# Nerozud/dl_reference_models

Hardware: NVIDIA B200
Metric: agent_steps_per_sec (higher is better)
Workload: dtype int16/u8

## Files before the change

dl_reference_models_b200/csrc/mapf_env_kernel.cuh:

```cuda
#pragma once

#include "mapf_kernels.cuh"

namespace mapf {

constexpr int ENV_MAX_ROWS = 64;
constexpr int ENV_T1_OFF = 0;
constexpr int ENV_KTH_OFF = 512;
constexpr int ENV_FREEROW_OFF = 768;
constexpr int ENV_FREEBITS_OFF = 1024;
constexpr int ENV_GDT_OFF = 1280;
constexpr int ENV_LUT_OFF = 2048;
constexpr int ENV_ROW_PAD = 2;

__host__ __device__ constexpr int env_stage_stride(int V2) { return ((4 * V2 + 20 + 3) / 4) | 1; }
__host__ __device__ constexpr int env_stage_bytes(int V2) {
    return 32 * env_stage_stride(V2) * 4 > 32 * 64 ? 32 * env_stage_stride(V2) * 4 : 32 * 64;
}

struct EnvLayout {
    int tables_bytes;
    int pre_off;
    int warp_bytes;
    int board_rows;
    int nq;
    int total_bytes;
};

__host__ __device__ inline EnvLayout make_env_layout(int N, int R, int C, int SR, int fw, int warps) {
    const int V = 2 * SR + 1, V2 = V * V;
    EnvLayout E;
    E.pre_off = (ENV_LUT_OFF + R * 32 * (V > 5 ? 8 : 4) + 15) & ~15;
    E.tables_bytes = E.pre_off + 65 * 4 + 12;
    E.board_rows = R > C ? R : C;
    if (N > E.board_rows) E.board_rows = N;
    E.board_rows += 2 * ENV_ROW_PAD;
    E.nq = (N + 3) / 4;
    int w = env_stage_bytes(V2);
    w += E.board_rows * 32 * 4;
    w += E.board_rows * 32 * 4;
    w += 4 * E.nq * 32 * 4;
    w = (w + 15) & ~15;
    E.warp_bytes = w;
    E.total_bytes = E.tables_bytes + w * warps + 1024;
    (void)fw;
    return E;
}

template <bool VEC>
__device__ __forceinline__ uint4 ldq32(const uint32_t *a, size_t i, int i0, int N, bool ok, uint32_t d) {
    uint4 v = make_uint4(d, d, d, d);
    if (VEC) { if (ok) v = *reinterpret_cast<const uint4 *>(a + i); }
    else if (ok) {
        if (i0 + 0 < N) v.x = a[i + 0];
        if (i0 + 1 < N) v.y = a[i + 1];
        if (i0 + 2 < N) v.z = a[i + 2];
        if (i0 + 3 < N) v.w = a[i + 3];
    }
    return v;
}
template <bool VEC>
__device__ __forceinline__ void stq32(uint32_t *a, size_t i, int i0, int N, bool ok, uint4 v) {
    if (!ok) return;
    if (VEC) *reinterpret_cast<uint4 *>(a + i) = v;
    else {
        if (i0 + 0 < N) a[i + 0] = v.x;
        if (i0 + 1 < N) a[i + 1] = v.y;
        if (i0 + 2 < N) a[i + 2] = v.z;
        if (i0 + 3 < N) a[i + 3] = v.w;
    }
}
template <bool VEC>
__device__ __forceinline__ uint32_t ldq8(const uint8_t *a, size_t i, int i0, int N, bool ok) {
    uint32_t v = 0;
    if (VEC) { if (ok) v = *reinterpret_cast<const uint32_t *>(a + i); }
    else if (ok) {
#pragma unroll
        for (int k = 0; k < 4; ++k) if (i0 + k < N) v |= (uint32_t)a[i + k] << (8 * k);
    }
    return v;
}
template <bool VEC>
__device__ __forceinline__ void stq8(uint8_t *a, size_t i, int i0, int N, bool ok, uint32_t v) {
    if (!ok) return;
    if (VEC) *reinterpret_cast<uint32_t *>(a + i) = v;
    else {
#pragma unroll
        for (int k = 0; k < 4; ++k) if (i0 + k < N) a[i + k] = (uint8_t)(v >> (8 * k));
    }
}
template <bool VEC>
__device__ __forceinline__ uint2 ldq16(const int16_t *a, size_t i, int i0, int N, bool ok) {
    uint2 v = make_uint2(0, 0);
    if (VEC) { if (ok) v = *reinterpret_cast<const uint2 *>(a + i); }
    else if (ok) {
        if (i0 + 0 < N) v.x |= (uint32_t)(uint16_t)a[i + 0];
        if (i0 + 1 < N) v.x |= (uint32_t)(uint16_t)a[i + 1] << 16;
        if (i0 + 2 < N) v.y |= (uint32_t)(uint16_t)a[i + 2];
        if (i0 + 3 < N) v.y |= (uint32_t)(uint16_t)a[i + 3] << 16;
    }
    return v;
}
template <bool VEC>
__device__ __forceinline__ void stq16(int16_t *a, size_t i, int i0, int N, bool ok, uint2 v) {
    if (!ok) return;
    if (VEC) *reinterpret_cast<uint2 *>(a + i) = v;
    else {
        if (i0 + 0 < N) a[i + 0] = (int16_t)(v.x & 0xFFFFu);
        if (i0 + 1 < N) a[i + 1] = (int16_t)(v.x >> 16);
        if (i0 + 2 < N) a[i + 2] = (int16_t)(v.y & 0xFFFFu);
        if (i0 + 3 < N) a[i + 3] = (int16_t)(v.y >> 16);
    }
}

__device__ __forceinline__ uint32_t qget(const uint4 &v, int k) { return k == 0 ? v.x : k == 1 ? v.y : k == 2 ? v.z : v.w; }
__device__ __forceinline__ void qset(uint4 &v, int k, uint32_t x) { if (k == 0) v.x = x; else if (k == 1) v.y = x; else if (k == 2) v.z = x; else v.w = x; }
__device__ __forceinline__ uint32_t hget(const uint2 &v, int k) { const uint32_t w = (k < 2) ? v.x : v.y; return (k & 1) ? (w >> 16) : (w & 0xFFFFu); }
__device__ __forceinline__ void hset(uint2 &v, int k, uint32_t x) {
    uint32_t &w = (k < 2) ? v.x : v.y;
    w = (k & 1) ? ((w & 0x0000FFFFu) | (x << 16)) : ((w & 0xFFFF0000u) | (x & 0xFFFFu));
}
__device__ __forceinline__ uint32_t code_of(uint32_t packed) { return ((packed & 0xFFFFu) << 5) | (packed >> 16); }
__device__ __forceinline__ uint32_t packed_of(uint32_t code) { return (code >> 5) | ((code & 31u) << 16); }

__device__ __forceinline__ uint4 sample_quad(unsigned long long seed, long long env_global, int quad,
                                             unsigned long long counter) {
    Philox ph(seed ^ 0xA511E9B3ull, env_global);
    return ph((uint32_t)counter, (uint32_t)(counter >> 32), (uint32_t)quad, 0x41435421u);
}

inline void build_env_tables(int SR, int R, int C, int wpr, int fw, const uint32_t *rows,
                             const uint32_t *free_bits, int normalize, float den0, float den1, unsigned char *img,
                             int pre_off) {
    const int V = 2 * SR + 1;
    {
        uint32_t *pre = reinterpret_cast<uint32_t *>(img + pre_off);
        uint32_t acc = 0;
        for (int w = 0; w <= 64; ++w) {
            pre[w] = acc;
            if (w < fw) acc += (uint32_t)__builtin_popcount(free_bits[w]);
        }
    }
    auto rowbits = [&](int r, int c0, int n) {
        unsigned long long x = 0;
        for (int j = 0; j < n; ++j) {
            const int bit = c0 + j + PAD;
            if ((rows[(r + PAD) * wpr + (bit >> 5)] >> (bit & 31)) & 1u) x |= 1ull << j;
        }
        return x;
    };
    uint32_t *t1 = reinterpret_cast<uint32_t *>(img + ENV_T1_OFF);
    for (int x = 0; x < (1 << V); ++x) {
        uint32_t s = 0;
        for (int j = 0; j < V; ++j) s |= ((uint32_t)(x >> j) & 1u) << (4 * j);
        t1[x] = s;
    }
    uint8_t *kth = img + ENV_KTH_OFF;
    for (int m = 0; m < 32; ++m)
        for (int k = 0; k < 8; ++k) {
            int pos = 0, seen = 0;
            for (int b = 0; b < 5; ++b)
                if ((m >> b) & 1) { if (seen == k) pos = b; ++seen; }
            kth[m * 8 + k] = (uint8_t)(k < seen ? pos : 0);
        }
    for (int cell = 0; cell < R * 32; ++cell) {
        const int r = cell >> 5, c = cell & 31;
        unsigned long long w = 0;
        if (c < C)
            for (int wr = 0; wr < V; ++wr) w |= rowbits(r - SR + wr, c - SR, V) << (wr * V);
        if (V > 5) reinterpret_cast<unsigned long long *>(img + ENV_LUT_OFF)[cell] = w;
        else reinterpret_cast<uint32_t *>(img + ENV_LUT_OFF)[cell] = (uint32_t)w;
    }
    uint32_t *freerow = reinterpret_cast<uint32_t *>(img + ENV_FREEROW_OFF);
    for (int r = 0; r < R; ++r) freerow[r] = (uint32_t)(~rowbits(r, 0, C) & (C >= 32 ? 0xFFFFFFFFull : ((1ull << C) - 1ull)));
    uint32_t *fb = reinterpret_cast<uint32_t *>(img + ENV_FREEBITS_OFF);
    for (int i = 0; i < fw; ++i) fb[i] = free_bits[i];
    float *gdt = reinterpret_cast<float *>(img + ENV_GDT_OFF);
    const int nr = 2 * R - 1, n = nr + 2 * C - 1;
    for (int i = 0; i < n; ++i) {
        const bool row = i < nr;
        const float d = (float)(row ? i - (R - 1) : i - nr - (C - 1));
        gdt[i] = normalize ? d / (row ? den0 : den1) : d;
    }
}

__device__ __forceinline__ uint32_t nibbles_to_bytes(uint32_t sel) {
    uint32_t w;
    asm("prmt.b32 %0, %1, %2, %3;" : "=r"(w) : "r"(0x03020100u), "r"(0x00000004u), "r"(sel));
    return w;
}
__device__ __forceinline__ uint32_t nibbles_to_bytes_0124(uint32_t sel) {
    uint32_t w;
    asm("prmt.b32 %0, %1, %2, %3;" : "=r"(w) : "r"(0x04020100u), "r"(0u), "r"(sel));
    return w;
}
__device__ __forceinline__ uint32_t spread4(uint32_t m) { return ((m & 15u) * 0x00204081u) & 0x01010101u; }
__device__ __forceinline__ uint32_t gather4(uint32_t w, int b) { return ((((w >> b) & 0x01010101u) * 0x01020408u) >> 24) & 15u; }
__device__ __forceinline__ int action_delta(uint32_t a) { return (int)(int8_t)__byte_perm(0x2001E000u, 0x000000FFu, a); }
__device__ __forceinline__ uint32_t lds_pure(uint32_t saddr) {
    uint32_t v;
    asm("ld.shared.u32 %0, [%1];" : "=r"(v) : "r"(saddr));
    return v;
}
__device__ __forceinline__ uint32_t lds_pure(uint32_t saddr, uint32_t tag) {
    uint32_t v;
    asm("{ .reg .b32 t; mov.b32 t, %2; ld.shared.u32 %0, [%1]; }" : "=r"(v) : "r"(saddr), "r"(tag));
    return v;
}
__device__ __forceinline__ uint32_t lds_pure_u8(uint32_t saddr) {
    uint32_t v;
    asm("ld.shared.u8 %0, [%1];" : "=r"(v) : "r"(saddr));
    return v;
}
template <typename WB> __device__ __forceinline__ WB lut_ld(uint32_t saddr);
template <> __device__ __forceinline__ uint32_t lut_ld<uint32_t>(uint32_t saddr) { return lds_pure(saddr); }
template <> __device__ __forceinline__ unsigned long long lut_ld<unsigned long long>(uint32_t saddr) {
    unsigned long long v;
    asm("ld.shared.u64 %0, [%1];" : "=l"(v) : "r"(saddr));
    return v;
}
__device__ __forceinline__ void sts_stage(uint32_t saddr, uint32_t v) {
    asm volatile("st.shared.u32 [%0], %1;" ::"r"(saddr), "r"(v));
}

__device__ __forceinline__ void sts_stage_u8(uint32_t saddr, uint32_t v) {
    asm volatile("st.shared.u8 [%0], %1;" ::"r"(saddr), "r"(v));
}

constexpr uint32_t REC_CODE = 0x7FFu;

template <int SR, bool VEC, bool FAST = false, bool MANY = false>
__global__ void __launch_bounds__(448, 1) mapf_step_env_kernel(const KParams p, const EnvLayout E) {
    const bool kLifelong = FAST ? true : p.lifelong;
    const bool kLock = FAST ? true : p.lock_enabled;
    constexpr int V = 2 * SR + 1, V2 = V * V;
    constexpr uint32_t VM = (1u << V) - 1u;
    constexpr uint32_t M4 = VM << 2;
    constexpr int OBS_W = V2;
    constexpr int STRIDE = env_stage_stride(V2);
    constexpr int STAGE_BYTES = env_stage_bytes(V2);
    constexpr int CTR = SR * V + SR;
    constexpr int PADR = ENV_ROW_PAD;
    using WB = typename WinBits<V>::type;
    extern __shared__ __align__(16) unsigned char esm[];
    const unsigned full = 0xFFFFFFFFu;
    const int tid = threadIdx.x, lane = tid & 31, warp = tid >> 5, warps = blockDim.x >> 5;
    const int N = p.N, R = p.R, C = p.C, NQ = E.nq;

    {
        const uint4 *src = reinterpret_cast<const uint4 *>(p.env_tables);
        uint4 *dst = reinterpret_cast<uint4 *>(esm);
        for (int i = tid; i < (E.tables_bytes >> 4); i += blockDim.x) dst[i] = src[i];
    }
    asm volatile("griddepcontrol.launch_dependents;");
    if (p.env_prefetch) {
        const int tile0 = blockIdx.x * (blockDim.x >> 5) + (tid >> 5);
        const int left = p.B - tile0 * 32;
        if (left > 0) {
            const size_t a0 = (size_t)tile0 * 32 * (size_t)p.N;
            const uint32_t agents = (uint32_t)(left < 32 ? left : 32) * (uint32_t)p.N;
            const void *ptr = nullptr;
            uint32_t bytes = agents * 4u;
            switch (tid & 31) {
                case 0: ptr = p.positions + a0; break;
                case 1: ptr = p.goals + a0; break;
                case 2: ptr = p.lock_gp + a0; break;
                case 3: ptr = p.lock_mv + a0; break;
                case 4: ptr = p.lock_fm + a0; break;
                case 5: ptr = p.actions ? p.actions + a0 : nullptr; bytes = agents; break;
                case 6: ptr = p.agent_flags + a0; bytes = agents; break;
                case 7: ptr = p.env_words + (size_t)tile0 * 32 * 4; bytes = (uint32_t)(left < 32 ? left : 32) * 64u; break;
                default: break;
            }
            bytes &= ~15u;
            if (ptr && bytes && (reinterpret_cast<uintptr_t>(ptr) & 15) == 0)
                asm volatile("cp.async.bulk.prefetch.L2.global [%0], %1;" ::"l"(ptr), "r"(bytes) : "memory");
        }
    }
    asm volatile("griddepcontrol.wait;" ::: "memory");
    __syncthreads();
    const char *t1b = reinterpret_cast<const char *>(esm + ENV_T1_OFF);
    const uint8_t *kth = esm + ENV_KTH_OFF;
    const WB *lut = reinterpret_cast<const WB *>(esm + ENV_LUT_OFF);
    const uint32_t *freerow = reinterpret_cast<const uint32_t *>(esm + ENV_FREEROW_OFF);
    const uint32_t *freebits = reinterpret_cast<const uint32_t *>(esm + ENV_FREEBITS_OFF);
    const float *gdt = reinterpret_cast<const float *>(esm + ENV_GDT_OFF);
    const uint32_t esm_s = (uint32_t)__cvta_generic_to_shared(esm);
    const uint32_t t1_s = esm_s + ENV_T1_OFF, kth_s = esm_s + ENV_KTH_OFF, lut_s = esm_s + ENV_LUT_OFF;
    const uint32_t *freepre = reinterpret_cast<const uint32_t *>(esm + E.pre_off);
    auto kth_free = [&](int k) -> int {
        int lo = 0;
#pragma unroll
        for (int stp = 32; stp >= 1; stp >>= 1)
            if (lo + stp < p.fw && (int)freepre[lo + stp] <= k) lo += stp;
        return lo * 32 + (int)__fns(freebits[lo], 0, k - (int)freepre[lo] + 1);
    };

    unsigned char *wsm = esm + E.tables_bytes + warp * E.warp_bytes;
    uint32_t *stage_w = reinterpret_cast<uint32_t *>(wsm);
    uint32_t *my_stage = stage_w + lane * STRIDE;
    const uint32_t my_stage_s = (uint32_t)__cvta_generic_to_shared(my_stage);
    uint32_t *occ_w = reinterpret_cast<uint32_t *>(wsm + STAGE_BYTES);
    uint32_t *goal_w = occ_w + E.board_rows * 32;
    uint32_t *rec_w = goal_w + E.board_rows * 32;
    uint32_t *occ = occ_w + lane, *goalb = goal_w + lane, *rec = rec_w + lane;
    const uint32_t goalb_s = (uint32_t)__cvta_generic_to_shared(goalb);
    uint32_t *rowm = occ, *colm = goalb;
    const int ntiles = (p.B + 31) / 32;
    uint32_t errs = 0;
    const uint32_t mdw = p.dw >= 32 ? full : ((1u << p.dw) - 1u);
    const uint32_t mlw = p.lw >= 32 ? full : ((1u << p.lw) - 1u);
    const uint32_t allN = (N >= 32) ? full : ((1u << N) - 1u);

    auto emit_final = [&](size_t abe, size_t oo, unsigned long long sctr, long long eg, const uint32_t *occ_e,
                          const uint32_t *goal_e, uint32_t code, uint32_t gcode, uint32_t bp_bit, bool ctr2) {
        if (lane >= N) return;
        const int r = (int)(code >> 5), c = (int)(code & 31u);
        const WB obst = lut[code];
        const int sa = c > SR ? c - SR : 0, sb2 = (c < SR ? SR - c : 0) + 2;
        const uint32_t *orow = occ_e + (r - SR) * 32, *grow = goal_e + (r - SR) * 32;
        uint32_t acc[(4 * V2 + 31) / 32 + 1];
#pragma unroll
        for (int j = 0; j < (int)(sizeof(acc) / sizeof(acc[0])); ++j) acc[j] = 0;
        uint32_t blk_up = 0, blk_mid = 0, blk_dn = 0;
#pragma unroll
        for (int wr = 0; wr < V; ++wr) {
            const uint32_t bx = orow[wr * 32], by = grow[wr * 32];
            const uint32_t o4 = (wr * V >= 2 ? (uint32_t)(obst >> (wr * V - 2)) : (uint32_t)(obst << 2)) & M4;
            const uint32_t MC = (wr == SR) ? (M4 & ~(4u << SR)) : M4;
            const uint32_t occ4 = ((bx >> sa) << sb2) & MC;
            const uint32_t agent4 = occ4 & ~o4, blk4 = occ4 | o4;
            const uint32_t g4 = ((by >> sa) << sb2) & M4 & ~blk4;
            if (wr == SR - 1) blk_up = blk4;
            if (wr == SR) blk_mid = blk4;
            if (wr == SR + 1) blk_dn = blk4;
            const uint32_t t = *reinterpret_cast<const uint32_t *>(t1b + o4) +
                               (*reinterpret_cast<const uint32_t *>(t1b + agent4) << 1) +
                               (*reinterpret_cast<const uint32_t *>(t1b + g4) << 2);
            const int bitpos = 4 * V * wr, wi = bitpos >> 5, sh = bitpos & 31;
            acc[wi] |= t << sh;
            if (sh + 4 * V > 32) acc[wi + 1] |= t >> (32 - sh);
        }
        const uint32_t am = 1u | ((~blk_up >> (2 + SR)) & 1u) << 1 | ((~blk_mid >> (2 + SR + 1)) & 1u) << 2 |
                            ((~blk_dn >> (2 + SR)) & 1u) << 3 | ((~blk_mid >> (2 + SR - 1)) & 1u) << 4;
        if (p.o_local_obs) {
            uint8_t *ob = p.o_local_obs + (abe + oo + lane) * V2;
#pragma unroll
            for (int n = 0; n < V2; ++n) ob[n] = (uint8_t)((acc[n >> 3] >> (4 * (n & 7))) & 0xFu);
            const int dr = (int)(gcode >> 5) - r + SR, dc = (int)(gcode & 31u) - c + SR;
            if ((unsigned)dr < (unsigned)V && (unsigned)dc < (unsigned)V) {
                const int ci = dr * V + dc;
                const bool occ_other = (ci != CTR) && ((occ_e[(gcode >> 5) * 32] >> (gcode & 31u)) & 1u);
                if (!((obst >> ci) & 1) && !occ_other) ob[ci] = 3;
            }
            if (ctr2) ob[CTR] = 2;
        }
        if (p.o_action_mask) {
#pragma unroll
            for (int k = 0; k < 5; ++k) p.o_action_mask[(abe + oo + lane) * 5 + k] = (int8_t)((am >> k) & 1u);
        }
        if (p.o_goal_delta) {
            const int gi0 = (int)(gcode >> 5) - r + (R - 1), gi1 = (int)(gcode & 31u) - c + (C - 1) + 2 * R - 1;
            p.o_goal_delta[abe + oo + lane] = make_float2(gdt[gi0], gdt[gi1]);
        }
        if (p.o_blocking_prev) p.o_blocking_prev[abe + oo + lane] = (uint8_t)bp_bit;
        if (p.sample_mode) {
            const uint4 rnd = sample_quad(p.seed, eg, lane >> 2, sctr);
            const uint32_t x = qget(rnd, lane & 3);
            const uint32_t na = p.sample_mode == 1 ? kth[am * 8 + __umulhi(x, (uint32_t)__popc(am))] : __umulhi(x, 5u);
            p.o_next_actions[abe + lane] = (int8_t)na;
        }
    };

    for (int tile = blockIdx.x * warps + warp; tile < ntiles; tile += gridDim.x * warps) {
    const int env = tile * 32 + lane;
    const bool ok = env < p.B;
    const size_t ab = (size_t)(ok ? env : 0) * N;
    const long long env_global = p.env_id_base + env;
    const size_t env0 = (size_t)tile * 32;
    for (int it = 0; it < (MANY ? p.inner_steps : 1); ++it) {
    const size_t so = MANY ? (size_t)it * (size_t)p.out_step_stride : 0, oo = so * (size_t)N;
    const unsigned long long sctr = p.sample_counter + (MANY ? (unsigned long long)it : 0ull);
    const int8_t *acts_in = (MANY && it > 0) ? p.o_next_actions : p.actions;

    int lock_count = 0, lock_head = 0;
    if (ok) {
        const int *ew1 = reinterpret_cast<const int *>(p.env_words + (size_t)env * 4);
        lock_count = ew1[MAPF_W_LOCK_COUNT];
        lock_head = ew1[MAPF_W_LOCK_HEAD];
    }
    const int count_after = lock_count + 1;
    if (lock_head < 0 || lock_head >= p.lw) lock_head = 0;
    const int slot_new = lock_head;
    const int slot_next = (lock_head + 1 == p.lw) ? 0 : lock_head + 1;
    const bool use_ring = kLock && count_after >= p.lw && p.lw > 1;

    uint32_t reached_m = 0, completed_m = 0, bprev_m = 0;
    bool degen = false;
    uint32_t solo_m = 0xFFFFFFFFu;
    for (int r = 0; r < E.board_rows; ++r) { occ[r * 32] = 0u; goalb[r * 32] = 0u; }
    uint32_t dup = 0;
    auto prepass_quad = [&](int i0, const uint4 &pq, const uint4 &gq, uint32_t act4, uint32_t fl4) {
        reached_m |= gather4(fl4, 0) << i0;
        completed_m |= gather4(fl4, 1) << i0;
        bprev_m |= gather4(fl4, 2) << i0;
        solo_m &= ~(gather4(fl4, 3) << i0);
#pragma unroll
        for (int k = 0; k < 4; ++k) {
            if (VEC || i0 + k < N) {
                const uint32_t code = code_of(qget(pq, k)), gcode = code_of(qget(gq, k));
                int a = (int)(int8_t)(act4 >> (8 * k));
                if (a < 0 || a > 4) { errs |= MAPF_DEV_ERR_INVALID_ACTION; a = 0; }
                const uint32_t nbi = __byte_perm((uint32_t)CTR | ((uint32_t)(CTR - V) << 8) | ((uint32_t)(CTR + 1) << 16) |
                                                 ((uint32_t)(CTR + V) << 24), (uint32_t)(CTR - 1), (uint32_t)a) & 0xFFu;
                const uint32_t tblocked = ((uint32_t)lut[code] >> nbi) & 1u;
                rec[(i0 + k) * 32] = code | ((uint32_t)a << 11) | (tblocked << 14) | (gcode << 16);
                if (ok) {
                    if (!((fl4 >> (8 * k + 3)) & 1u)) {
                        const uint32_t cb0 = 1u << (code & 31u);
                        dup |= atomicOr(&occ[(code >> 5) * 32], cb0) & cb0;
                    } else degen = true;
                    atomicOr(&goalb[(gcode >> 5) * 32], 1u << (gcode & 31u));
                }
            }
        }
    };
    for (int q = 0; q < NQ; q += 2) {
        const int i0 = 4 * q, i1 = i0 + 4;
        const bool two = q + 1 < NQ;
        const uint4 pq0 = ldq32<VEC>(p.positions, ab + i0, i0, N, ok, 0u);
        const uint4 gq0 = ldq32<VEC>(p.goals, ab + i0, i0, N, ok, 0u);
        const uint32_t ac0 = acts_in ? ldq8<VEC>(reinterpret_cast<const uint8_t *>(acts_in), ab + i0, i0, N, ok) : 0u;
        const uint32_t fl0 = ldq8<VEC>(p.agent_flags, ab + i0, i0, N, ok);
        const uint4 pq1 = ldq32<VEC>(p.positions, ab + i1, i1, N, ok && two, 0u);
        const uint4 gq1 = ldq32<VEC>(p.goals, ab + i1, i1, N, ok && two, 0u);
        const uint32_t ac1 = acts_in ? ldq8<VEC>(reinterpret_cast<const uint8_t *>(acts_in), ab + i1, i1, N, ok && two) : 0u;
        const uint32_t fl1 = ldq8<VEC>(p.agent_flags, ab + i1, i1, N, ok && two);
        prepass_quad(i0, pq0, gq0, ac0, fl0);
        if (two) prepass_quad(i1, pq1, gq1, ac1, fl1);
    }
    degen |= dup != 0;
    if (degen) {
        const uint32_t claim = solo_m;
        for (int i = 0; i < N; ++i)
            for (int j = i + 1; j < N; ++j)
                if (((claim >> j) & 1u) && ((rec[i * 32] ^ rec[j * 32]) & REC_CODE) == 0u) { solo_m &= ~(1u << i); break; }
    }

    uint32_t moved_m = 0, failed_m = 0, gstep_m = 0, ongoal_m = 0;
    uint32_t Gd = 0, Md = 0, Fd = 0, Gl = 0, Ml = 0;
    const unsigned act_w = __ballot_sync(full, ok);
    const bool masked_sampler = p.sample_mode == 1;

    uint4 gp_n = make_uint4(0, 0, 0, 0), mv_n = gp_n, fm_n = gp_n;
    uint2 ring_n = make_uint2(0u, 0u);
    auto load_lock = [&](int i0) {
        if (!kLock) return;
        gp_n = ldq32<VEC>(p.lock_gp, ab + i0, i0, N, ok, 0u);
        mv_n = ldq32<VEC>(p.lock_mv, ab + i0, i0, N, ok, 0u);
        fm_n = ldq32<VEC>(p.lock_fm, ab + i0, i0, N, ok, 0u);
        if (use_ring) ring_n = ldq16<VEC>(p.lock_dist, ((size_t)(ok ? env : 0) * p.lw + slot_next) * N + i0, i0, N, ok);
    };
    load_lock(0);
    for (int q = 0; q < NQ; ++q) {
        const int i0 = 4 * q;
        uint32_t rv4[4];
#pragma unroll
        for (int k = 0; k < 4; ++k) rv4[k] = (VEC || i0 + k < N) ? rec[(i0 + k) * 32] : 0u;
        uint4 gpq = gp_n, mvq = mv_n, fmq = fm_n;
        const uint2 ringq = ring_n;
        uint4 rnd = make_uint4(0, 0, 0, 0);
        if (p.sample_mode) rnd = sample_quad(p.seed, env_global, q, sctr);
        uint32_t ds[4] = {0, 0, 0, 0}, cd[4] = {0, 0, 0, 0}, gc[4] = {0, 0, 0, 0};
        uint32_t masks4 = 0, next4 = 0;
        int patch[4];
        uint32_t win[4][V];
#pragma unroll
        for (int k = 0; k < 4; ++k) {
            patch[k] = 4 * V2 + 20;
#pragma unroll
            for (int wr = 0; wr < V; ++wr) win[k][wr] = 0;
            if (!VEC && i0 + k >= N) continue;
            const uint32_t bit = 1u << (i0 + k);
            uint32_t code = rv4[k] & REC_CODE;
            const uint32_t gcode = rv4[k] >> 16;
            const uint32_t ocode = code;
            const uint32_t a = (rv4[k] >> 11) & 7u;
            const uint32_t tcode = code + (uint32_t)action_delta(a);
            const bool wants = ok && a != 0 && !(rv4[k] & 0x4000u);
            const uint32_t tb = 1u << (tcode & 31u);
            const uint32_t tv = occ[(tcode >> 5) * 32];
            const bool moves = wants & ((tv & tb) == 0u);
            atomicAnd(&occ[(code >> 5) * 32], moves ? ~(1u << (code & 31u)) : 0xFFFFFFFFu);
            atomicOr(&occ[(tcode >> 5) * 32], moves ? tb : 0u);
            const bool failed = ok && a != 0 && !moves;
            moved_m |= moves ? bit : 0u;
            failed_m |= failed ? bit : 0u;
            code = moves ? tcode : code;
            const bool on_goal = ok && code == gcode;
            bool gstep = false, cur_on_goal = on_goal;
            if (!kLifelong) {
                if (on_goal && !(reached_m & bit)) { reached_m |= bit; completed_m |= bit; gstep = true; }
            } else if (on_goal) {
                gstep = true;
                completed_m |= bit; reached_m &= ~bit;
                cur_on_goal = false;
            }
            gstep_m |= gstep ? bit : 0u;
            ongoal_m |= cur_on_goal ? bit : 0u;
            uint32_t delta16 = 0;
            if (kLock) {
                const bool prev_on_goal = kLifelong ? false : (ocode == gcode);
                const bool gp = kLifelong ? gstep : (!prev_on_goal && cur_on_goal);
                const uint32_t g2 = (qget(gpq, k) << 1) | (gp ? 1u : 0u);
                const uint32_t m2 = (qget(mvq, k) << 1) | (moves ? 1u : 0u);
                const uint32_t f2 = (qget(fmq, k) << 1) | (failed ? 1u : 0u);
                qset(gpq, k, g2); qset(mvq, k, m2); qset(fmq, k, f2);
                const uint32_t okbit = ok ? bit : 0u;
                Gd |= (g2 & mdw) ? okbit : 0u;
                Md |= (m2 & mdw) ? okbit : 0u;
                Fd |= (f2 & mdw) ? okbit : 0u;
                Gl |= (g2 & mlw) ? okbit : 0u;
                Ml |= (m2 & mlw) ? okbit : 0u;
                const int dist = abs((int)(gcode >> 5) - (int)(code >> 5)) + abs((int)(gcode & 31u) - (int)(code & 31u));
                ds[k] = (uint32_t)dist;
                delta16 = (use_ring && ok) ? (uint32_t)((int)(int16_t)hget(ringq, k) - dist) << 16 : 0u;
            }
            rec[(i0 + k) * 32] = code | (rv4[k] & 0x7800u) | delta16;
            cd[k] = code;
            gc[k] = gcode;
            const int r = (int)(code >> 5), c = (int)(code & 31u);
            const WB obst = lut_ld<WB>(lut_s + code * (uint32_t)sizeof(WB));
            const int sa = c > SR ? c - SR : 0, sb2 = (c < SR ? SR - c : 0) + 2;
            const uint32_t *orow = &occ[(r - SR) * 32];
            const uint32_t grow_s = goalb_s + (uint32_t)((r - SR) * 128);
            uint32_t blk_up = 0, blk_mid = 0, blk_dn = 0;
#pragma unroll
            for (int wr = 0; wr < V; ++wr) {
                const uint32_t bx = orow[wr * 32];
                const uint32_t by = lds_pure(grow_s + (uint32_t)(wr * 128), (uint32_t)tile);
                const uint32_t o4 = (wr * V >= 2 ? (uint32_t)(obst >> (wr * V - 2)) : (uint32_t)(obst << 2)) & M4;
                const uint32_t MC = (wr == SR) ? (M4 & ~(4u << SR)) : M4;
                const uint32_t occ4 = ((bx >> sa) << sb2) & MC;
                const uint32_t agent4 = occ4 & ~o4;
                const uint32_t blk4 = occ4 | o4;
                const uint32_t g4 = ((by >> sa) << sb2) & M4 & ~blk4;
                if (wr == SR - 1) blk_up = blk4;
                if (wr == SR) blk_mid = blk4;
                if (wr == SR + 1) blk_dn = blk4;
                win[k][wr] = lds_pure(t1_s + (o4 | g4)) + (lds_pure(t1_s + (agent4 | g4)) << 1);
            }
            const uint32_t am = 1u | ((~blk_up >> (2 + SR)) & 1u) << 1 | ((~blk_mid >> (2 + SR + 1)) & 1u) << 2 |
                                ((~blk_dn >> (2 + SR)) & 1u) << 3 | ((~blk_mid >> (2 + SR - 1)) & 1u) << 4;
            masks4 |= am << (8 * k);
            {
                const int dr = (int)(gcode >> 5) - r + SR, dc = (int)(gcode & 31u) - c + SR;
                const bool in = (unsigned)dr < (unsigned)V && (unsigned)dc < (unsigned)V;
                const int ci = in ? dr * V + dc : 0;
                const bool occ_other = (ci != CTR) && ((occ[(gcode >> 5) * 32] >> (gcode & 31u)) & 1u);
                patch[k] = (in && !((obst >> ci) & 1) && !occ_other) ? V2 * k + ci : 4 * V2 + 20;
            }
            {
                const uint32_t x = qget(rnd, k);
                const uint32_t na_masked = lds_pure_u8(kth_s + am * 8u + __umulhi(x, (uint32_t)__popc(am)));
                const uint32_t na = masked_sampler ? na_masked : __umulhi(x, 5u);
                next4 |= na << (8 * k);
            }
        }
        stq32<VEC>(p.positions, ab + i0, i0, N, ok,
                   make_uint4(packed_of(cd[0]), packed_of(cd[1]), packed_of(cd[2]), packed_of(cd[3])));
        if (kLock) {
            stq32<VEC>(p.lock_gp, ab + i0, i0, N, ok, gpq);
            stq32<VEC>(p.lock_mv, ab + i0, i0, N, ok, mvq);
            stq32<VEC>(p.lock_fm, ab + i0, i0, N, ok, fmq);
            stq16<VEC>(p.lock_dist, ((size_t)(ok ? env : 0) * p.lw + slot_new) * N + i0, i0, N, ok,
                       make_uint2(ds[0] | (ds[1] << 16), ds[2] | (ds[3] << 16)));
        }
        if (q + 1 < NQ) load_lock(i0 + 4);
        uint32_t carry = 0;
#pragma unroll
        for (int k = 0; k < 4; ++k) {
            if (!VEC && i0 + k >= N) continue;
            uint32_t acc[(4 * (V2 + 3) + 31) / 32 + 1];
#pragma unroll
            for (int j = 0; j < (int)(sizeof(acc) / sizeof(acc[0])); ++j) acc[j] = 0;
#pragma unroll
            for (int wr = 0; wr < V; ++wr) {
                const uint32_t t = win[k][wr];
                const int bitpos = 4 * (V * wr + (k & 3));
                const int wi = bitpos >> 5, sh = bitpos & 31;
                acc[wi] |= t << sh;
                if (sh + 4 * V > 32) acc[wi + 1] |= t >> (32 - sh);
            }
            constexpr int NWMAX = (V2 + 3 + 3) / 4;
            const int j0 = (V2 * k) >> 2;
            const int nw = ((k & 3) + V2 + 3) >> 2;
#pragma unroll
            for (int m = 0; m < NWMAX; ++m) {
                if (m >= nw) continue;
                uint32_t w = nibbles_to_bytes_0124((m & 1) ? (acc[m >> 1] >> 16) : acc[m >> 1]);
                if (m == 0 && (k & 3) != 0) w |= carry;
                if (m == nw - 1 && (((k & 3) + V2) & 3) != 0) carry = w;
                else sts_stage(my_stage_s + (uint32_t)((j0 + m) * 4), w);
            }
            if (!VEC && i0 + k == N - 1 && (((k & 3) + V2) & 3) != 0) sts_stage(my_stage_s + (uint32_t)((j0 + nw - 1) * 4), carry);
        }
        {
#pragma unroll
            for (int k = 0; k < 4; ++k) sts_stage_u8(my_stage_s + (uint32_t)patch[k], 3u);
            uint32_t lo[4], hi[4];
#pragma unroll
            for (int k = 0; k < 4; ++k) {
                const uint32_t m = (masks4 >> (8 * k)) & 0x1Fu;
                lo[k] = spread4(m);
                hi[k] = m >> 4;
            }
            my_stage[OBS_W + 0] = lo[0];
            my_stage[OBS_W + 1] = hi[0] | (lo[1] << 8);
            my_stage[OBS_W + 2] = (lo[1] >> 24) | (hi[1] << 8) | (lo[2] << 16);
            my_stage[OBS_W + 3] = (lo[2] >> 16) | (hi[2] << 16) | (lo[3] << 24);
            my_stage[OBS_W + 4] = (lo[3] >> 8) | (hi[3] << 24);
        }
        if (ok) {
            if (p.o_goal_delta) {
                float2 gd[4];
#pragma unroll
                for (int k = 0; k < 4; ++k) {
                    const int gi0 = (int)(gc[k] >> 5) - (int)(cd[k] >> 5) + (R - 1);
                    const int gi1 = (int)(gc[k] & 31u) - (int)(cd[k] & 31u) + (C - 1) + 2 * R - 1;
                    gd[k] = (VEC || i0 + k < N) ? make_float2(gdt[gi0], gdt[gi1]) : make_float2(0.f, 0.f);
                }
                if (VEC) {
                    asm volatile("st.global.v8.f32 [%0], {%1,%2,%3,%4,%5,%6,%7,%8};" ::"l"(p.o_goal_delta + ab + oo + i0),
                                 "f"(gd[0].x), "f"(gd[0].y), "f"(gd[1].x), "f"(gd[1].y), "f"(gd[2].x), "f"(gd[2].y),
                                 "f"(gd[3].x), "f"(gd[3].y) : "memory");
                } else {
#pragma unroll
                    for (int k = 0; k < 4; ++k) if (i0 + k < N) p.o_goal_delta[ab + oo + i0 + k] = gd[k];
                }
            }
            if (p.o_blocking_prev) stq8<VEC>(p.o_blocking_prev, ab + oo + i0, i0, N, true, spread4(bprev_m >> i0));
            if (p.sample_mode) stq8<VEC>(reinterpret_cast<uint8_t *>(p.o_next_actions), ab + i0, i0, N, true, next4);
        }
        __syncwarp();
        if (VEC) {
            const size_t agent0 = env0 * N + oo + (size_t)i0;
            for (int w = lane; w < OBS_W + 5; w += 32) {
                const bool is_obs = w < OBS_W;
                unsigned char *gp = is_obs ? (p.o_local_obs ? p.o_local_obs + agent0 * V2 + 4 * w : nullptr)
                                           : (p.o_action_mask ? reinterpret_cast<unsigned char *>(p.o_action_mask) +
                                                                    agent0 * 5 + 4 * (w - OBS_W) : nullptr);
                const uint32_t gstride = (uint32_t)N * (uint32_t)(is_obs ? V2 : 5);
                const uint32_t *src = stage_w + w;
                if (gp) {
                    if (act_w == full) {
#pragma unroll
                        for (int e = 0; e < 32; ++e)
                            *reinterpret_cast<uint32_t *>(gp + (size_t)e * gstride) = src[e * STRIDE];
                    } else {
#pragma unroll 1
                        for (int e = 0; e < 32; ++e)
                            if ((act_w >> e) & 1u)
                                *reinterpret_cast<uint32_t *>(gp + (size_t)e * gstride) = src[e * STRIDE];
                    }
                }
            }
        } else {
            const int na = (N - i0) < 4 ? (N - i0) : 4;
            for (int e = 0; e < 32; ++e) {
                if (!((act_w >> e) & 1u)) continue;
                const uint8_t *src = reinterpret_cast<const uint8_t *>(stage_w + e * STRIDE);
                if (p.o_local_obs) {
                    uint8_t *dst = p.o_local_obs + ((env0 + e) * N + oo + i0) * V2;
                    for (int b = lane; b < na * V2; b += 32) dst[b] = src[b];
                }
                if (p.o_action_mask) {
                    uint8_t *dst = reinterpret_cast<uint8_t *>(p.o_action_mask) + ((env0 + e) * N + oo + i0) * 5;
                    for (int b = lane; b < na * 5; b += 32) dst[b] = src[4 * OBS_W + b];
                }
            }
        }
        __syncwarp();
    }

    const uint32_t ew_s = (uint32_t)__cvta_generic_to_shared(stage_w) + (uint32_t)lane * 16u;
    {
        const int4 *src = p.env_words + (size_t)(ok ? env : 0) * 4;
#pragma unroll
        for (int k = 0; k < 4; ++k)
            asm volatile("cp.async.cg.shared.global [%0], [%1], 16, %2;" ::"r"(ew_s + 512u * k), "l"(src + k),
                         "r"(ok ? 16 : 0) : "memory");
        asm volatile("cp.async.commit_group;" ::: "memory");
    }
    int *ew_slot = reinterpret_cast<int *>(stage_w) + lane * 4;
    auto ew_ld = [&](int word) -> int { return ew_slot[128 * (word >> 2) + (word & 3)]; };

    if (__any_sync(full, degen)) {
        __syncwarp();
        if (degen && ok) {
            for (int i = 0; i < N; ++i) {
                const uint32_t rvi = rec[i * 32], newc = rvi & REC_CODE, biti = 1u << i;
                const bool mvd = (moved_m >> i) & 1u;
                const uint32_t oldc = mvd ? newc - (uint32_t)action_delta((rvi >> 11) & 7u) : newc;
                bool owned_by_other = false;
                for (int a2 = 0; a2 < N; ++a2) {
                    if (a2 == i) continue;
                    const uint32_t rva = rec[a2 * 32];
                    uint32_t ca = rva & REC_CODE;
                    if (a2 > i && ((moved_m >> a2) & 1u)) ca -= (uint32_t)action_delta((rva >> 11) & 7u);
                    if (ca == oldc) {
                        if (mvd) solo_m &= ~(1u << a2);
                        else if ((solo_m >> a2) & 1u) owned_by_other = true;
                    }
                }
                if (mvd) solo_m |= biti;
                else if (!(solo_m & biti) && owned_by_other && p.o_local_obs)
                    p.o_local_obs[(ab + oo + i) * V2 + CTR] = 2;
            }
        }
        __syncwarp();
    }

    if (kLock) lock_head = slot_next;
    const int arrivals = __popc(gstep_m);
    const uint32_t pend = kLifelong ? gstep_m : 0u;
    const bool reassigned = pend != 0;
    {
        unsigned rw = __ballot_sync(full, pend != 0);
        if (rw) asm volatile("cp.async.wait_all;" ::: "memory");
        const uint32_t rng_counter0 = rw ? (uint32_t)ew_ld(MAPF_W_RNG_COUNTER) : 0u;
        while (rw) {
            const int e = __ffs(rw) - 1;
            rw &= rw - 1;
            uint32_t pe = __shfl_sync(full, pend, e);
            const uint32_t mv_e = __shfl_sync(full, moved_m, e), bp_e = __shfl_sync(full, bprev_m, e);
            const uint32_t solo_e = __shfl_sync(full, degen ? solo_m : 0xFFFFFFFFu, e);
            const uint32_t rc_e = __shfl_sync(full, rng_counter0, e);
            const int slot_new_e = __shfl_sync(full, slot_new, e), slot_next_e = __shfl_sync(full, slot_next, e);
            const bool use_ring_e = __shfl_sync(full, (int)use_ring, e) != 0;
            const long long eg = p.env_id_base + (long long)(env0 + e);
            const size_t abe = (env0 + e) * (size_t)N, enve = env0 + e;
            uint32_t *occ_e = occ_w + e, *goal_e = goal_w + e, *rec_e = rec_w + e;
            uint32_t rng_inc = 0, err_e = 0, ongoal_fix = 0;
            while (pe) {
                const int i = __ffs(pe) - 1;
                pe &= pe - 1;
                const uint32_t later = mv_e & ~((2u << i) - 1u);
                const bool und = lane < N && ((later >> lane) & 1u);
                uint32_t nc = 0, oc = 0;
                if (und) {
                    const uint32_t rv = rec_e[lane * 32];
                    nc = rv & REC_CODE;
                    oc = nc - (uint32_t)action_delta((rv >> 11) & 7u);
                    atomicAnd(&occ_e[(nc >> 5) * 32], ~(1u << (nc & 31u)));
                }
                const uint32_t gold = code_of(p.goals[abe + i]);
                if (lane == 0) goal_e[(gold >> 5) * 32] &= ~(1u << (gold & 31u));
                __syncwarp();
                if (und) atomicOr(&occ_e[(oc >> 5) * 32], 1u << (oc & 31u));
                __syncwarp();
                uint32_t ng = 0xFFFFFFFFu;
                if (p.goal_override) {
                    const uint32_t ov = p.goal_override[abe + i];
                    if (prow(ov) >= 0) ng = code_of(ov);
                }
                if (ng == 0xFFFFFFFFu) {
                    const uint32_t c0 = lane < R ? (freerow[lane] & ~occ_e[lane * 32] & ~goal_e[lane * 32]) : 0u;
                    const uint32_t c1 = lane + 32 < R ? (freerow[lane + 32] & ~occ_e[(lane + 32) * 32] & ~goal_e[(lane + 32) * 32]) : 0u;
                    const int n0 = __popc(c0), n1 = __popc(c1);
                    int pre0 = n0, pre1 = n1;
#pragma unroll
                    for (int sft = 1; sft < 32; sft <<= 1) {
                        const int v0 = __shfl_up_sync(full, pre0, sft), v1 = __shfl_up_sync(full, pre1, sft);
                        if (lane >= sft) { pre0 += v0; pre1 += v1; }
                    }
                    const int tot0 = __shfl_sync(full, pre0, 31), n = tot0 + __shfl_sync(full, pre1, 31);
                    int kk = -1;
                    if (p.goal_rank) kk = p.goal_rank[abe + i];
                    if (kk < 0 && n > 0) {
                        const Philox ph(p.seed, eg);
                        const uint4 x = ph(rc_e + rng_inc, (uint32_t)i, 0x474F414Cu , 0);
                        kk = (int)__umulhi(x.x, (uint32_t)n);
                        rng_inc++;
                    }
                    if (n > 0 && kk < n) {
                        const bool hit0 = kk >= pre0 - n0 && kk < pre0;
                        const bool hit1 = kk >= tot0 + pre1 - n1 && kk < tot0 + pre1;
                        uint32_t mine = 0;
                        if (hit0) mine = (uint32_t)(lane * 32) + __fns(c0, 0, kk - (pre0 - n0) + 1);
                        if (hit1) mine = (uint32_t)((lane + 32) * 32) + __fns(c1, 0, kk - tot0 - (pre1 - n1) + 1);
                        const unsigned hb = __ballot_sync(full, hit0 || hit1);
                        ng = __shfl_sync(full, mine, __ffs(hb) - 1);
                    } else {
                        err_e |= MAPF_DEV_ERR_NO_GOAL_CELL;
                    }
                }
                if (ng == 0xFFFFFFFFu) { ng = gold; ongoal_fix |= 1u << i; }
                if (lane == 0) {
                    goal_e[(ng >> 5) * 32] |= 1u << (ng & 31u);
                    p.goals[abe + i] = packed_of(ng);
                    if (kLock) {
                        const uint32_t rv = rec_e[i * 32], code = rv & REC_CODE;
                        const int dist = abs((int)(ng >> 5) - (int)(code >> 5)) + abs((int)(ng & 31u) - (int)(code & 31u));
                        p.lock_dist[((size_t)enve * p.lw + slot_new_e) * N + i] = (int16_t)dist;
                        if (use_ring_e) {
                            const int ring_old = (int)p.lock_dist[((size_t)enve * p.lw + slot_next_e) * N + i];
                            rec_e[i * 32] = (rv & 0xFFFFu) | ((uint32_t)(ring_old - dist) << 16);
                        }
                    }
                }
                if (und) atomicAnd(&occ_e[(oc >> 5) * 32], ~(1u << (oc & 31u)));
                __syncwarp();
                if (und) atomicOr(&occ_e[(nc >> 5) * 32], 1u << (nc & 31u));
                __syncwarp();
            }
            {
                const uint32_t code = lane < N ? (rec_e[lane * 32] & REC_CODE) : 0u;
                const uint32_t gcode = lane < N ? code_of(p.goals[abe + lane]) : 0u;
                const bool ctr2 = !((solo_e >> lane) & 1u) && ((occ_e[(code >> 5) * 32] >> (code & 31u)) & 1u);
                emit_final(abe, oo, sctr, eg, occ_e, goal_e, code, gcode, (bp_e >> lane) & 1u, ctr2);
            }
            if (lane == e) {
                ew_slot[128 * (MAPF_W_RNG_COUNTER >> 2) + (MAPF_W_RNG_COUNTER & 3)] = (int)(rc_e + rng_inc);
                errs |= err_e; ongoal_m |= ongoal_fix;
            }
            __syncwarp();
        }
    }

    __syncwarp();
    constexpr bool PK = FAST;
    uint32_t todo = ok ? allN : 0u;
    if (PK) {
        for (int r = 0; r < E.board_rows; ++r) goalb[r * 32] = 0u;
        uint32_t near_m = 0;
        if (ok) {
#pragma unroll 1
            for (int i = 0; i < N; ++i) {
                const uint32_t code = rec[i * 32] & REC_CODE;
                const int r = (int)(code >> 5);
                atomicOr(&goalb[(r + PADR) * 32], 1u << i);
                atomicOr(&goalb[((code & 31u) + PADR) * 32], 0x10000u << i);
                const uint32_t *orow = &occ[(r - 2) * 32];
                const uint32_t b = 1u << (code & 31u);
                const uint32_t m1 = (b << 1) | (b >> 1), mB = m1 | b, mA = m1 | (b << 2) | (b >> 2);
                const uint32_t nr = (orow[64] & mA) | ((orow[32] | orow[96]) & mB) | ((orow[0] | orow[128]) & b);
                near_m |= nr ? (1u << i) : 0u;
            }
        }
        todo = (p.nearby == 2 && !degen && reached_m == 0u) ? (near_m | failed_m) & todo : todo;
    } else {
        for (int r = 0; r < E.board_rows; ++r) { occ[r * 32] = 0u; goalb[r * 32] = 0u; }
        if (ok) {
#pragma unroll 1
            for (int i = 0; i < N; ++i) {
                const uint32_t code = rec[i * 32] & REC_CODE;
                atomicOr(&rowm[((code >> 5) + PADR) * 32], 1u << i);
                atomicOr(&colm[((code & 31u) + PADR) * 32], 1u << i);
            }
        }
    }
    auto rowset = [&](int idx) -> uint32_t { return PK ? (goalb[idx * 32] & 0xFFFFu) : rowm[idx * 32]; };
    auto colset = [&](int idx) -> uint32_t { return PK ? (goalb[idx * 32] >> 16) : colm[idx * 32]; };
    uint32_t coloc_any = 0, wf_alive = 0, flags_any = 0;
    uint32_t wf_m = 0, blocking_m = 0;
    const uint32_t intent_m = allN & ~reached_m;
#pragma unroll 1
    while (todo) {
        const int i = __ffs(todo) - 1;
        todo &= todo - 1;
        const uint32_t bit = 1u << i;
        const uint32_t rv = rec[i * 32];
        const uint32_t code = rv & REC_CODE;
        const int r = (int)(code >> 5), c = (int)(code & 31u);
        const int pr = r + PADR, pc = c + PADR;
        const uint32_t row0 = rowset(pr), col0 = colset(pc);
        const uint32_t here = row0 & col0;
        if (here & ~bit) coloc_any |= bit;
        if (kLock && !(ongoal_m & bit)) {
            uint32_t nb = 0;
            if (p.nearby == 2) {
                const uint32_t c1 = col0 | colset(pc - 1) | colset(pc + 1);
                const uint32_t c2 = c1 | colset(pc - 2) | colset(pc + 2);
                nb = (row0 & c2) | ((rowset(pr - 1) | rowset(pr + 1)) & c1) | ((rowset(pr - 2) | rowset(pr + 2)) & col0);
            } else {
                uint32_t u = 0;
                for (int w = 0; w <= p.nearby; ++w) {
                    const int dd = p.nearby - w;
                    if (c - w >= 0) u |= colset(pc - w);
                    if (c + w < C) u |= colset(pc + w);
                    uint32_t rm = 0;
                    if (r - dd >= 0) rm |= rowset(pr - dd);
                    if (r + dd < R) rm |= rowset(pr + dd);
                    nb |= rm & u;
                }
            }
            nb &= ~here;
            if (__popc(nb) >= p.min_nb) {
                const uint32_t P = nb | bit;
                if (!(P & Gd) && !(P & Md) && (P & Fd)) flags_any |= 1u;
                if (!(P & Gl) && (P & Ml)) {
                    uint32_t rest = nb;
                    int red = (int)rv >> 16;
                    while (rest) {
                        const int a = __ffs(rest) - 1;
                        rest &= rest - 1;
                        red += (int)rec[a * 32] >> 16;
                    }
                    if (red <= p.eps_floor) flags_any |= 2u;
                }
            }
        }
// ... 235 lines not shown
```

Before: 17.53 billion.

## Rewrite window extraction with funnel-shift rotation and fewer shared-memory lookups

Replaces the per-row shift pair with a single funnel-shift rotation and folds the obstacle, agent and goal masks into two table lookups whose shared base is carried in the address bits. The 5-bit action mask is now derived with one multiply-gather. The goal patch check moves from an occupancy/obstacle test to a read-compare-write on the staged byte. A Manhattan distance is computed with __sad. It also adds opaque asm on the Philox keys and realigns shared memory to 1024 bytes so OR-based address formation works. The aim is fewer ALU ops and shared loads per window row, at the cost of an added shared read per patch and reliance on alignment assumptions.

```diff
diff --git a/dl_reference_models_b200/csrc/mapf_env_kernel.cuh b/dl_reference_models_b200/csrc/mapf_env_kernel.cuh
--- a/dl_reference_models_b200/csrc/mapf_env_kernel.cuh
+++ b/dl_reference_models_b200/csrc/mapf_env_kernel.cuh
@@ -126,6 +126,8 @@
 __device__ __forceinline__ uint4 sample_quad(unsigned long long seed, long long env_global, int quad,
                                              unsigned long long counter) {
     Philox ph(seed ^ 0xA511E9B3ull, env_global);
+    asm("{ .reg .b32 t; mov.b32 t, %1; }" : "+r"(ph.k1) : "r"(quad));
+    asm("{ .reg .b32 t; mov.b32 t, %1; }" : "+r"(ph.k0) : "r"(quad));
     return ph((uint32_t)counter, (uint32_t)(counter >> 32), (uint32_t)quad, 0x41435421u);
 }
 
@@ -219,12 +221,35 @@
     asm("ld.shared.u64 %0, [%1];" : "=l"(v) : "r"(saddr));
     return v;
 }
+template <int SR>
+__device__ __forceinline__ uint32_t window_row(uint32_t bx, uint32_t by, uint32_t o4, uint32_t rot, uint32_t MC,
+                                               uint32_t t1_s, uint32_t &blk4) {
+    constexpr uint32_t M4 = ((1u << (2 * SR + 1)) - 1u) << 2;
+    const uint32_t occ4 = __funnelshift_r(bx, bx, rot) & MC;
+    const uint32_t gb = (__funnelshift_r(by, by, rot) & M4) | t1_s;
+    blk4 = occ4 | o4;
+    return lds_pure(o4 | (gb & ~occ4)) + (lds_pure((occ4 | gb) & ~o4) << 1);
+}
+
+template <int SR>
+__device__ __forceinline__ uint32_t action_mask(uint32_t up, uint32_t mid, uint32_t dn) {
+    constexpr uint32_t NB = (1u << (2 + SR)) | (1u << (10 + SR)) | (1u << (19 + SR)) | (1u << (17 + SR));
+    constexpr uint32_t GATHER = (1u << (26 - SR)) | (1u << (20 - SR)) | (1u << (10 - SR)) | (1u << (14 - SR));
+    const uint32_t w = up + (dn << 8) + (mid << 16);
+    return ((((~w & NB) * GATHER) >> 27) & 0x1Eu) | 1u;
+}
+
 __device__ __forceinline__ void sts_stage(uint32_t saddr, uint32_t v) {
     asm volatile("st.shared.u32 [%0], %1;" ::"r"(saddr), "r"(v));
 }
 
 __device__ __forceinline__ void sts_stage_u8(uint32_t saddr, uint32_t v) {
     asm volatile("st.shared.u8 [%0], %1;" ::"r"(saddr), "r"(v));
+}
+__device__ __forceinline__ uint32_t lds_stage_u8(uint32_t saddr) {
+    uint32_t v;
+    asm volatile("ld.shared.u8 %0, [%1];" : "=r"(v) : "r"(saddr));
+    return v;
 }
 
 constexpr uint32_t REC_CODE = 0x7FFu;
@@ -242,14 +267,14 @@
     constexpr int CTR = SR * V + SR;
     constexpr int PADR = ENV_ROW_PAD;
     using WB = typename WinBits<V>::type;
-    extern __shared__ __align__(16) unsigned char esm[];
+    extern __shared__ __align__(1024) unsigned char env_sm[];
     const unsigned full = 0xFFFFFFFFu;
     const int tid = threadIdx.x, lane = tid & 31, warp = tid >> 5, warps = blockDim.x >> 5;
     const int N = p.N, R = p.R, C = p.C, NQ = E.nq;
 
     {
         const uint4 *src = reinterpret_cast<const uint4 *>(p.env_tables);
-        uint4 *dst = reinterpret_cast<uint4 *>(esm);
+        uint4 *dst = reinterpret_cast<uint4 *>(env_sm);
         for (int i = tid; i < (E.tables_bytes >> 4); i += blockDim.x) dst[i] = src[i];
     }
     asm volatile("griddepcontrol.launch_dependents;");
@@ -279,15 +304,14 @@
     }
     asm volatile("griddepcontrol.wait;" ::: "memory");
     __syncthreads();
-    const char *t1b = reinterpret_cast<const char *>(esm + ENV_T1_OFF);
-    const uint8_t *kth = esm + ENV_KTH_OFF;
-    const WB *lut = reinterpret_cast<const WB *>(esm + ENV_LUT_OFF);
-    const uint32_t *freerow = reinterpret_cast<const uint32_t *>(esm + ENV_FREEROW_OFF);
-    const uint32_t *freebits = reinterpret_cast<const uint32_t *>(esm + ENV_FREEBITS_OFF);
-    const float *gdt = reinterpret_cast<const float *>(esm + ENV_GDT_OFF);
-    const uint32_t esm_s = (uint32_t)__cvta_generic_to_shared(esm);
+    const uint8_t *kth = env_sm + ENV_KTH_OFF;
+    const WB *lut = reinterpret_cast<const WB *>(env_sm + ENV_LUT_OFF);
+    const uint32_t *freerow = reinterpret_cast<const uint32_t *>(env_sm + ENV_FREEROW_OFF);
+    const uint32_t *freebits = reinterpret_cast<const uint32_t *>(env_sm + ENV_FREEBITS_OFF);
+    const float *gdt = reinterpret_cast<const float *>(env_sm + ENV_GDT_OFF);
+    const uint32_t esm_s = (uint32_t)__cvta_generic_to_shared(env_sm);
     const uint32_t t1_s = esm_s + ENV_T1_OFF, kth_s = esm_s + ENV_KTH_OFF, lut_s = esm_s + ENV_LUT_OFF;
-    const uint32_t *freepre = reinterpret_cast<const uint32_t *>(esm + E.pre_off);
+    const uint32_t *freepre = reinterpret_cast<const uint32_t *>(env_sm + E.pre_off);
     auto kth_free = [&](int k) -> int {
         int lo = 0;
 #pragma unroll
@@ -296,7 +320,7 @@
         return lo * 32 + (int)__fns(freebits[lo], 0, k - (int)freepre[lo] + 1);
     };
 
-    unsigned char *wsm = esm + E.tables_bytes + warp * E.warp_bytes;
+    unsigned char *wsm = env_sm + E.tables_bytes + warp * E.warp_bytes;
     uint32_t *stage_w = reinterpret_cast<uint32_t *>(wsm);
     uint32_t *my_stage = stage_w + lane * STRIDE;
     const uint32_t my_stage_s = (uint32_t)__cvta_generic_to_shared(my_stage);
@@ -317,7 +341,7 @@
         if (lane >= N) return;
         const int r = (int)(code >> 5), c = (int)(code & 31u);
         const WB obst = lut[code];
-        const int sa = c > SR ? c - SR : 0, sb2 = (c < SR ? SR - c : 0) + 2;
+        const uint32_t rot = (uint32_t)(c - SR - 2) & 31u;
         const uint32_t *orow = occ_e + (r - SR) * 32, *grow = goal_e + (r - SR) * 32;
         uint32_t acc[(4 * V2 + 31) / 32 + 1];
 #pragma unroll
@@ -328,21 +352,17 @@
             const uint32_t bx = orow[wr * 32], by = grow[wr * 32];
             const uint32_t o4 = (wr * V >= 2 ? (uint32_t)(obst >> (wr * V - 2)) : (uint32_t)(obst << 2)) & M4;
             const uint32_t MC = (wr == SR) ? (M4 & ~(4u << SR)) : M4;
-            const uint32_t occ4 = ((bx >> sa) << sb2) & MC;
-            const uint32_t agent4 = occ4 & ~o4, blk4 = occ4 | o4;
-            const uint32_t g4 = ((by >> sa) << sb2) & M4 & ~blk4;
+            uint32_t blk4;
+            uint32_t t = window_row<SR>(bx, by, o4, rot, MC, t1_s, blk4);
+            t += t & (t >> 1) & 0x11111111u;
             if (wr == SR - 1) blk_up = blk4;
             if (wr == SR) blk_mid = blk4;
             if (wr == SR + 1) blk_dn = blk4;
-            const uint32_t t = *reinterpret_cast<const uint32_t *>(t1b + o4) +
-                               (*reinterpret_cast<const uint32_t *>(t1b + agent4) << 1) +
-                               (*reinterpret_cast<const uint32_t *>(t1b + g4) << 2);
             const int bitpos = 4 * V * wr, wi = bitpos >> 5, sh = bitpos & 31;
             acc[wi] |= t << sh;
             if (sh + 4 * V > 32) acc[wi + 1] |= t >> (32 - sh);
         }
-        const uint32_t am = 1u | ((~blk_up >> (2 + SR)) & 1u) << 1 | ((~blk_mid >> (2 + SR + 1)) & 1u) << 2 |
-                            ((~blk_dn >> (2 + SR)) & 1u) << 3 | ((~blk_mid >> (2 + SR - 1)) & 1u) << 4;
+        const uint32_t am = action_mask<SR>(blk_up, blk_mid, blk_dn);
         if (p.o_local_obs) {
             uint8_t *ob = p.o_local_obs + (abe + oo + lane) * V2;
 #pragma unroll
@@ -522,16 +542,16 @@
                 Fd |= (f2 & mdw) ? okbit : 0u;
                 Gl |= (g2 & mlw) ? okbit : 0u;
                 Ml |= (m2 & mlw) ? okbit : 0u;
-                const int dist = abs((int)(gcode >> 5) - (int)(code >> 5)) + abs((int)(gcode & 31u) - (int)(code & 31u));
-                ds[k] = (uint32_t)dist;
-                delta16 = (use_ring && ok) ? (uint32_t)((int)(int16_t)hget(ringq, k) - dist) << 16 : 0u;
+                const uint32_t dist = __sad((int)(gcode >> 5), (int)(code >> 5), __sad((int)(gcode & 31u), (int)(code & 31u), 0u));
+                ds[k] = dist;
+                delta16 = (use_ring && ok) ? (uint32_t)((int)(int16_t)hget(ringq, k) - (int)dist) << 16 : 0u;
             }
             rec[(i0 + k) * 32] = code | (rv4[k] & 0x7800u) | delta16;
             cd[k] = code;
             gc[k] = gcode;
             const int r = (int)(code >> 5), c = (int)(code & 31u);
             const WB obst = lut_ld<WB>(lut_s + code * (uint32_t)sizeof(WB));
-            const int sa = c > SR ? c - SR : 0, sb2 = (c < SR ? SR - c : 0) + 2;
+            const uint32_t rot = (uint32_t)(c - SR - 2) & 31u;
             const uint32_t *orow = &occ[(r - SR) * 32];
             const uint32_t grow_s = goalb_s + (uint32_t)((r - SR) * 128);
             uint32_t blk_up = 0, blk_mid = 0, blk_dn = 0;
@@ -541,24 +561,18 @@
                 const uint32_t by = lds_pure(grow_s + (uint32_t)(wr * 128), (uint32_t)tile);
                 const uint32_t o4 = (wr * V >= 2 ? (uint32_t)(obst >> (wr * V - 2)) : (uint32_t)(obst << 2)) & M4;
                 const uint32_t MC = (wr == SR) ? (M4 & ~(4u << SR)) : M4;
-                const uint32_t occ4 = ((bx >> sa) << sb2) & MC;
-                const uint32_t agent4 = occ4 & ~o4;
-                const uint32_t blk4 = occ4 | o4;
-                const uint32_t g4 = ((by >> sa) << sb2) & M4 & ~blk4;
+                uint32_t blk4;
+                win[k][wr] = window_row<SR>(bx, by, o4, rot, MC, t1_s, blk4);
                 if (wr == SR - 1) blk_up = blk4;
                 if (wr == SR) blk_mid = blk4;
                 if (wr == SR + 1) blk_dn = blk4;
-                win[k][wr] = lds_pure(t1_s + (o4 | g4)) + (lds_pure(t1_s + (agent4 | g4)) << 1);
-            }
-            const uint32_t am = 1u | ((~blk_up >> (2 + SR)) & 1u) << 1 | ((~blk_mid >> (2 + SR + 1)) & 1u) << 2 |
-                                ((~blk_dn >> (2 + SR)) & 1u) << 3 | ((~blk_mid >> (2 + SR - 1)) & 1u) << 4;
+            }
+            const uint32_t am = action_mask<SR>(blk_up, blk_mid, blk_dn);
             masks4 |= am << (8 * k);
             {
                 const int dr = (int)(gcode >> 5) - r + SR, dc = (int)(gcode & 31u) - c + SR;
                 const bool in = (unsigned)dr < (unsigned)V && (unsigned)dc < (unsigned)V;
-                const int ci = in ? dr * V + dc : 0;
-                const bool occ_other = (ci != CTR) && ((occ[(gcode >> 5) * 32] >> (gcode & 31u)) & 1u);
-                patch[k] = (in && !((obst >> ci) & 1) && !occ_other) ? V2 * k + ci : 4 * V2 + 20;
+                patch[k] = in ? V2 * k + dr * V + dc : 4 * V2 + 20;
             }
             {
                 const uint32_t x = qget(rnd, k);
@@ -607,7 +621,10 @@
         }
         {
 #pragma unroll
-            for (int k = 0; k < 4; ++k) sts_stage_u8(my_stage_s + (uint32_t)patch[k], 3u);
+            for (int k = 0; k < 4; ++k) {
+                const uint32_t pa = my_stage_s + (uint32_t)patch[k];
+                if (lds_stage_u8(pa) == 4u) sts_stage_u8(pa, 3u);
+            }
             uint32_t lo[4], hi[4];
 #pragma unroll
             for (int k = 0; k < 4; ++k) {
```

Measured after the change: 17.50 billion, median of 6. Within noise of the previous version (-0.2%).
